# iwbn/flow-supervisor

Measured on AMD Instinct MI355X. Metric: image-pairs/s fwd+bwd, 12 GRU iters, 436x1024, higher is better.
Workload: dtype f32 (bf16x3 products); 1 GPU; RAFT full, 440x1024 (Sintel 436x1024 padded), 12 GRU iters, 4 pairs/GPU, train step = fwd + sequence loss + bwd + RCCL all-reduce + clip + AdamW; global_batch=4, parallelism=dp1, launch=hipGraph replay of the whole step

## Files before the change

flow_supervisor_amd/csrc/conv_igemm.hip:

```cpp
#include "conv_common.hpp"

namespace {

__device__ __forceinline__ void tile_of_block(int swz, int& bx, int& by) {
  if (!swz) return;
  const int nx = gridDim.x, T = nx * gridDim.y, i = by * nx + bx;
  const int x = i & 7, q = T >> 3, r = T & 7;
  const int t = x * q + (x < r ? x : r) + (i >> 3);
  bx = t % nx; by = t / nx;
}

template <class Cfg>
struct ConvALoader {
  static constexpr int BM = Cfg::BM, BK = Cfg::BK, LD = Cfg::LDA;
  static constexpr int F4 = BK / 4;
  static constexpr int NF4 = BM * F4 / 256;
  static constexpr int NREG = NF4 * 4;
  static constexpr int NCH = NF4;
  const float* p0; const float* p1; const float* p2;
  int C0, C1, C2, ld0, ld1, ld2;
  int cpt0, cpt1, cpt2;
  int taps, KW, PH, PW, H, W;
  int py[NF4], px[NF4];
  int64_t pb[NF4];
  __device__ __forceinline__ bool fetch_chunk(int kt, float (&r)[NREG], int j) const {
    const int n0 = taps * cpt0, n1 = taps * cpt1;
    const bool is1 = kt >= n0, is2 = kt >= n0 + n1;
    const int k = kt - (is1 ? n0 : 0) - (is2 ? n1 : 0);
    const int C = C0 + (is1 ? C1 - C0 : 0) + (is2 ? C2 - C1 : 0);
    const int ld = ld0 + (is1 ? ld1 - ld0 : 0) + (is2 ? ld2 - ld1 : 0);
    const int cpt = cpt0 + (is1 ? cpt1 - cpt0 : 0) + (is2 ? cpt2 - cpt1 : 0);
    const float* p = p0 + (is1 ? p1 - p0 : 0) + (is2 ? p2 - p1 : 0);
    const int tap = k / cpt, c0 = (k % cpt) * BK;
    const int dy = tap / KW - PH, dx = tap % KW - PW;
    const int kq = (threadIdx.x + 256 * j) % F4;
    const int yy = py[j] + dy, xx = px[j] + dx, c = c0 + kq * 4;
    const bool ok = py[j] >= 0 && yy >= 0 && yy < H && xx >= 0 && xx < W && c < C;
    const f32x4 v = gload4(p + (ok ? (pb[j] + (int64_t)yy * W + xx) * ld + c : 0));
    r[4 * j + 0] = v[0]; r[4 * j + 1] = v[1]; r[4 * j + 2] = v[2]; r[4 * j + 3] = v[3];
    return ok;
  }
  __device__ __forceinline__ void store_chunk(float* t, const float (&r)[NREG], int j, bool ok) const {
    const int e = threadIdx.x + 256 * j;
    const int row = e / F4, kq = e % F4;
#pragma unroll
    for (int c = 0; c < 4; ++c) t[(kq * 4 + c) * LD + row] = ok ? r[4 * j + c] : 0.f;
  }
};

template <class Cfg>
struct SplitConvALoader {
  static constexpr int NCH = Cfg::NCH_A, NREG = NCH * 4;
  const float* p0; const float* p1; const float* p2;
  int C0, C1, C2, ld0, ld1, ld2, cpt0, cpt1, cpt2;
  int taps, KW, PH, PW, H, W;
  int py[NCH], px[NCH];
  int pofs[NCH];
  __device__ __forceinline__ void fetch_chunk(int kt, float (&r)[NREG], int j) const {
    const int n0 = taps * cpt0, n1 = taps * cpt1;
    const bool is1 = kt >= n0, is2 = kt >= n0 + n1;
    const int k = kt - (is1 ? n0 : 0) - (is2 ? n1 : 0);
    const int C = C0 + (is1 ? C1 - C0 : 0) + (is2 ? C2 - C1 : 0);
    const int ld = ld0 + (is1 ? ld1 - ld0 : 0) + (is2 ? ld2 - ld1 : 0);
    const int cpt = cpt0 + (is1 ? cpt1 - cpt0 : 0) + (is2 ? cpt2 - cpt1 : 0);
    const float* p = p0 + (is1 ? p1 - p0 : 0) + (is2 ? p2 - p1 : 0);
    const int tap = k / cpt, c0 = (k % cpt) * 32;
    const int dy = tap / KW - PH, dx = tap % KW - PW;
    const int kq = (threadIdx.x + 256 * j) & 7;
    const int c = c0 + kq * 4;
    const bool ok = ((unsigned)(py[j] + dy) < (unsigned)H) && ((unsigned)(px[j] + dx) < (unsigned)W) && c < C;
    const float* src = ok ? p + (int64_t)(pofs[j] + dy * W + dx) * ld + c : g_fsraft_zero16;
    const f32x4 v = gload4(src);
    r[4 * j + 0] = v[0]; r[4 * j + 1] = v[1]; r[4 * j + 2] = v[2]; r[4 * j + 3] = v[3];
  }
  __device__ __forceinline__ void stage_chunk(char* tile, const float* r4, int j) const {
    stage_convert<Cfg::PITCH>(tile, threadIdx.x + 256 * j, r4);
  }
};

template <class Cfg>
struct BufConvALoader {
  static constexpr int NCH = Cfg::NCH_A, NREG = NCH * 4;
  const float* b0; const float* b1; const float* b2; unsigned nb0, nb1, nb2;
  unsigned ld0x4, ld1x4, ld2x4;
  const unsigned __attribute__((address_space(4)))* ktab;
  unsigned tapmask[NCH];
  unsigned pofs[NCH];
  unsigned kq16;
  __device__ __forceinline__ void fetch_tile(int kt, float (&r)[NREG]) const {
    const unsigned e = ktab[__builtin_amdgcn_readfirstlane(kt)];
    const unsigned soff = (e & 0xffffu) << 4, tap = (e >> 16) & 15u, src = (e >> 20) & 3u, crem = (e >> 22) & 63u;
    const bool s1 = src >= 1, s2 = src >= 2;
    const unsigned ldb = ld0x4 + (s1 ? ld1x4 - ld0x4 : 0u) + (s2 ? ld2x4 - ld1x4 : 0u);
    const float* bp = b0 + (s1 ? b1 - b0 : 0) + (s2 ? b2 - b1 : 0);
    const __amdgpu_buffer_rsrc_t rs = make_rsrc(bp, 0x7fffffffu);
    const unsigned cok = kq16 < crem * 4u ? 1u : 0u;
#pragma unroll
    for (int j = 0; j < NCH; ++j) {
      const unsigned bad = (__builtin_amdgcn_ubfe(tapmask[j], tap, 1u) & cok) ^ 1u;
      const unsigned voff = (bad << 31) | (__umul24(pofs[j], ldb) + kq16);
      const u32x4 v = __builtin_amdgcn_raw_buffer_load_b128(rs, voff, soff, 0);
      const f32x4 f = __builtin_bit_cast(f32x4, v);
      r[4 * j + 0] = f[0]; r[4 * j + 1] = f[1]; r[4 * j + 2] = f[2]; r[4 * j + 3] = f[3];
    }
  }
  __device__ __forceinline__ void stage_chunk(char* tile, const float* r4, int j) const {
    stage_convert<Cfg::PITCH>(tile, threadIdx.x + Cfg::NT * j, r4);
  }
};

template <class Cfg>
struct BufConvALoaderU {
  static constexpr int NCH = Cfg::NCH_A, NREG = NCH * 4;
  const float* base;
  const unsigned __attribute__((address_space(4)))* ktab;
  unsigned tapmask[NCH];
  unsigned voff0[NCH];
  unsigned kq16;
  __device__ __forceinline__ void fetch_tile(int kt, float (&r)[NREG]) const {
    const int ku = __builtin_amdgcn_readfirstlane(kt);
    const unsigned soff = ktab[2 * ku], e = ktab[2 * ku + 1];
    const unsigned tap = e & 15u, crem4 = (e >> 4) * 4u;
    const __amdgpu_buffer_rsrc_t rs = make_rsrc(base, 0x7fffffffu);
    const unsigned cok = kq16 < crem4 ? 1u : 0u;
#pragma unroll
    for (int j = 0; j < NCH; ++j) {
      const unsigned bad = (__builtin_amdgcn_ubfe(tapmask[j], tap, 1u) & cok) ^ 1u;
      const u32x4 v = __builtin_amdgcn_raw_buffer_load_b128(rs, (bad << 31) | voff0[j], soff, 0);
      const f32x4 f = __builtin_bit_cast(f32x4, v);
      r[4 * j + 0] = f[0]; r[4 * j + 1] = f[1]; r[4 * j + 2] = f[2]; r[4 * j + 3] = f[3];
    }
  }
  __device__ __forceinline__ void stage_chunk(char* tile, const float* r4, int j) const {
    stage_convert<Cfg::PITCH>(tile, threadIdx.x + Cfg::NT * j, r4);
  }
};

template <class Cfg>
struct BufWeightLoader {
  static constexpr int NCH = Cfg::NCH_B, NREG = NCH * 4;
  const char* base; unsigned nbytes;
  unsigned voff[NCH];
  __device__ __forceinline__ void fetch_tile(int kt, float (&r)[NREG]) const {
    const int ku = __builtin_amdgcn_readfirstlane(kt);
    const __amdgpu_buffer_rsrc_t rs = make_rsrc(base, ku < 0 ? 0u : nbytes);
    const unsigned soff = ku < 0 ? 0u : (unsigned)ku * 128u;
#pragma unroll
    for (int j = 0; j < NCH; ++j) {
      const u32x4 v = __builtin_amdgcn_raw_buffer_load_b128(rs, voff[j], soff, 0);
      const f32x4 f = __builtin_bit_cast(f32x4, v);
      r[4 * j + 0] = f[0]; r[4 * j + 1] = f[1]; r[4 * j + 2] = f[2]; r[4 * j + 3] = f[3];
    }
  }
  __device__ __forceinline__ void stage_chunk(char* tile, const float* r4, int j) const {
    stage_copy<Cfg::PITCH>(tile, threadIdx.x + Cfg::NT * j, r4);
  }
};

template <class Cfg>
struct SplitWeightLoader {
  static constexpr int NCH = Cfg::NCH_B, NREG = NCH * 4;
  const char* base;
  int64_t row_bytes;
  int rows_valid;
  __device__ __forceinline__ void fetch_chunk(int kt, float (&r)[NREG], int j) const {
    const int e = threadIdx.x + 256 * j;
    const int row = e >> 3, part = e & 7;
    const char* src = (row < rows_valid && kt >= 0) ? base + row * row_bytes + (int64_t)kt * 128 + part * 16
                                                    : reinterpret_cast<const char*>(g_fsraft_zero16);
    const f32x4 v = gload4(src);
    r[4 * j + 0] = v[0]; r[4 * j + 1] = v[1]; r[4 * j + 2] = v[2]; r[4 * j + 3] = v[3];
  }
  __device__ __forceinline__ void stage_chunk(char* tile, const float* r4, int j) const {
    stage_copy<Cfg::PITCH>(tile, threadIdx.x + 256 * j, r4);
  }
};

template <class Cfg, int EPI>
__device__ __forceinline__ void conv_epilogue(const ConvArgs& a, f32x16 (&acc)[Cfg::TM][Cfg::TN], int m0, int n0) {
  const int HW = a.H * a.W;
  const int M = a.B * HW;
  const int lane = threadIdx.x & 63, wave = threadIdx.x >> 6;
#pragma unroll
  for (int nt = 0; nt < Cfg::TN; ++nt) {
    const int n = n0 + acc_col<Cfg>(nt);
    const bool nok = n < a.N;
    const float bias = (nok && a.bias) ? a.bias[n] : 0.f;
    int di = 0;
    if (a.ndst > 1 && n >= a.dst[1].n0) di = 1;
    if (a.ndst > 2 && n >= a.dst[2].n0) di = 2;
    float* dp = di == 0 ? a.dst[0].p : di == 1 ? a.dst[1].p : a.dst[2].p;
    const int64_t dbs = di == 0 ? a.dst[0].bs : di == 1 ? a.dst[1].bs : a.dst[2].bs;
    const int64_t dps = di == 0 ? a.dst[0].ps : di == 1 ? a.dst[1].ps : a.dst[2].ps;
    const int64_t dcs = di == 0 ? a.dst[0].cs : di == 1 ? a.dst[1].cs : a.dst[2].cs;
    const int dn0 = di == 0 ? a.dst[0].n0 : di == 1 ? a.dst[1].n0 : a.dst[2].n0;
    const bool dacc = (di == 0 ? a.dst[0].accumulate : di == 1 ? a.dst[1].accumulate : a.dst[2].accumulate) != 0;
    const float* mk = di == 0 ? a.rmask[0] : di == 1 ? a.rmask[1] : a.rmask[2];
    const int ldm = di == 0 ? a.ldmask[0] : di == 1 ? a.ldmask[1] : a.ldmask[2];
    const int mkc = di == 0 ? a.maskc[0] : di == 1 ? a.maskc[1] : a.maskc[2];
#pragma unroll
    for (int mt = 0; mt < Cfg::TM; ++mt) {
      const int mbase = m0 + (wave / Cfg::WN) * (Cfg::TM * 32) + mt * 32 + 4 * (lane >> 5);
      const int b0 = mbase / HW, pix0 = mbase - b0 * HW;
      if (EPI == EPI_PLAIN) {
#pragma unroll
        for (int hb = 0; hb < 2; ++hb) {
          int off[8];
#pragma unroll
          for (int q = 0; q < 8; ++q) {
            const int r = hb * 8 + q;
            const int d = (r & 3) + 8 * (r >> 2);
            int pix = pix0 + d, b = b0;
            if (pix >= HW) { pix -= HW; ++b; }
            const bool ok = nok && (mbase + d < M);
            off[q] = ok ? (int)(b * dbs + pix * dps + (n - dn0) * dcs) : -1;
          }
          float old[8];
#pragma unroll
          for (int q = 0; q < 8; ++q) old[q] = (dacc && off[q] >= 0) ? dp[off[q]] : 0.f;
#pragma unroll
          for (int q = 0; q < 8; ++q) {
            float v = (acc[mt][nt][hb * 8 + q] + bias) * a.alpha;
            if (a.relu) v = fmaxf(v, 0.f);
            v += old[q];
            if (off[q] >= 0 && mk && n - dn0 < mkc) {
              const int r = hb * 8 + q;
              const int64_t m = mbase + (r & 3) + 8 * (r >> 2);
              if (mk[m * ldm + (n - dn0)] <= 0.f) v = 0.f;
            }
            if (off[q] >= 0) dp[off[q]] = v;
          }
        }
      } else if (EPI == EPI_ZR) {
        const bool isz = n < a.hid;
        const int c = isz ? n : n - a.hid;
        float hh[16];
        bool ok[16];
#pragma unroll
        for (int r = 0; r < 16; ++r) {
          const int m = mbase + (r & 3) + 8 * (r >> 2);
          ok[r] = nok && m < M;
          hh[r] = (ok[r] && !isz) ? a.h[(int64_t)m * a.ldh + c] : 0.f;
        }
#pragma unroll
        for (int r = 0; r < 16; ++r) {
          const int64_t m = mbase + (r & 3) + 8 * (r >> 2);
          const float pre = (a.pre && ok[r]) ? a.pre[m * a.ldpre + n] : 0.f;
          const float sg = 1.0f / (1.0f + expf(-(acc[mt][nt][r] + bias + pre)));
          if (ok[r]) {
            if (isz) {
              a.dst[0].p[m * a.dst[0].ps + c] = sg;
            } else {
              a.aux2[m * a.ld2 + c] = sg;
              a.aux1[m * a.ld1 + c] = sg * hh[r];
            }
          }
        }
      } else {
        float hh[16], zz[16];
        bool ok[16];
#pragma unroll
        for (int r = 0; r < 16; ++r) {
          const int64_t m = mbase + (r & 3) + 8 * (r >> 2);
          ok[r] = nok && m < M;
          hh[r] = ok[r] ? a.h[m * a.ldh + n] : 0.f;
          zz[r] = ok[r] ? a.z[m * a.ldz + n] : 0.f;
        }
#pragma unroll
        for (int r = 0; r < 16; ++r) {
          const int64_t m = mbase + (r & 3) + 8 * (r >> 2);
          const float pre = (a.pre && ok[r]) ? a.pre[m * a.ldpre + n] : 0.f;
          const float q = tanhf(acc[mt][nt][r] + bias + pre);
          if (ok[r]) {
            a.aux1[m * a.ld1 + n] = q;
            a.dst[0].p[m * a.dst[0].ps + n] = (1.f - zz[r]) * hh[r] + zz[r] * q;
          }
        }
      }
    }
  }
}

template <class Cfg, int EPI, int NTW = Cfg::NT, bool PATCH = false>
__device__ __forceinline__ void conv_epilogue_lds(const ConvArgs& a, f32x16 (&acc)[Cfg::TM][Cfg::TN], int m0, int n0,
                                                  float* __restrict__ tile, bool owner = true, int pb = 0, int py0 = 0, int px0 = 0,
                                                  int64_t mofs = 0) {
  constexpr int LD = Cfg::BN + 4;
  const int HW = a.H * a.W;
  const int M = a.B * HW;
  const int lane = threadIdx.x & 63, wave = threadIdx.x >> 6;
  auto row_m = [&](int row) -> int64_t {
    if constexpr (PATCH) {
      const int y = py0 + (row >> 5), x = px0 + (row & 31);
      return (y < a.H && x < a.W) ? (int64_t)(pb * a.H + y) * a.W + x : -1;
    } else {
      return m0 + row < M ? (int64_t)m0 + row : -1;
    }
  };
  __syncthreads();
#pragma unroll
  for (int nt = 0; nt < Cfg::TN; ++nt) {
    const int nl = acc_col<Cfg>(nt);
    const float bias = (n0 + nl < a.N && a.bias) ? a.bias[n0 + nl] : 0.f;
#pragma unroll
    for (int mt = 0; mt < Cfg::TM; ++mt) {
      const int rbase = (wave / Cfg::WN) * (Cfg::TM * 32) + mt * 32 + 4 * (lane >> 5);
#pragma unroll
      for (int r = 0; r < 16; ++r) tile[(rbase + (r & 3) + 8 * (r >> 2)) * LD + nl] = acc[mt][nt][r] + bias;
    }
  }
  __syncthreads();
  constexpr int C4 = Cfg::BN / 4;
  constexpr int RPP = NTW / C4;
  (void)owner;
  const int c4 = threadIdx.x % C4, rsub = threadIdx.x / C4;
  const int n = n0 + c4 * 4;
  const bool stats = PATCH && EPI == EPI_PLAIN && a.st_sum != nullptr;
  if (n >= a.N && !stats) return;
  if (EPI == EPI_PLAIN) {
    f32x4 ssum = {0.f, 0.f, 0.f, 0.f}, ssq = {0.f, 0.f, 0.f, 0.f};
    if (n < a.N) {
    int di = 0;
    if (a.ndst > 1 && n >= a.dst[1].n0) di = 1;
    if (a.ndst > 2 && n >= a.dst[2].n0) di = 2;
    float* dp = di == 0 ? a.dst[0].p : di == 1 ? a.dst[1].p : a.dst[2].p;
    const int64_t dps = di == 0 ? a.dst[0].ps : di == 1 ? a.dst[1].ps : a.dst[2].ps;
    const int dn0 = di == 0 ? a.dst[0].n0 : di == 1 ? a.dst[1].n0 : a.dst[2].n0;
    const bool dacc = (di == 0 ? a.dst[0].accumulate : di == 1 ? a.dst[1].accumulate : a.dst[2].accumulate) != 0;
    const float* mk = di == 0 ? a.rmask[0] : di == 1 ? a.rmask[1] : a.rmask[2];
    const int ldm = di == 0 ? a.ldmask[0] : di == 1 ? a.ldmask[1] : a.ldmask[2];
    const int mkc = di == 0 ? a.maskc[0] : di == 1 ? a.maskc[1] : a.maskc[2];
    const int nv = a.N - n < 4 ? a.N - n : 4;
#pragma unroll 4
    for (int row = rsub; row < Cfg::BM; row += RPP) {
      const int64_t m = row_m(row);
      if (m < 0) { if (PATCH) continue; else break; }
      f32x4 v = *reinterpret_cast<const f32x4*>(tile + row * LD + c4 * 4);
      float* o = dp + (int64_t)(m + mofs) * dps + (n - dn0);
#pragma unroll
      for (int i = 0; i < 4; ++i) {
        v[i] *= a.alpha;
        if (a.relu) v[i] = fmaxf(v[i], 0.f);
      }
      if (nv == 4) {
        if (stats) { ssum += v; ssq += v * v; }
        if (dacc) {
          const f32x4 old = gload4(o);
#pragma unroll
          for (int i = 0; i < 4; ++i) v[i] += old[i];
        }
        if (mk) {
          const f32x4 y = gload4(mk + (int64_t)m * ldm + (n - dn0));
#pragma unroll
          for (int i = 0; i < 4; ++i) if (n - dn0 + i < mkc && y[i] <= 0.f) v[i] = 0.f;
        }
        gstore4(o, v);
      } else {
        for (int i = 0; i < nv; ++i) {
          float r = dacc ? gload1(o + i) + v[i] : v[i];
          if (mk && n - dn0 + i < mkc && gload1(mk + (int64_t)m * ldm + (n - dn0) + i) <= 0.f) r = 0.f;
          gstore1(o + i, r);
        }
      }
    }
    }
    if constexpr (PATCH) {
      if (stats) {
        __syncthreads();
        float* red = tile;
        *reinterpret_cast<f32x4*>(red + (rsub * Cfg::BN) + c4 * 4) = ssum;
        *reinterpret_cast<f32x4*>(red + ((RPP + rsub) * Cfg::BN) + c4 * 4) = ssq;
        __syncthreads();
        if (threadIdx.x < Cfg::BN && n0 + (int)threadIdx.x < a.N) {
          float t1 = 0.f, t2 = 0.f;
#pragma unroll 4
          for (int g = 0; g < RPP; ++g) { t1 += red[g * Cfg::BN + threadIdx.x]; t2 += red[(RPP + g) * Cfg::BN + threadIdx.x]; }
          const int64_t o = ((int64_t)pb * a.st_slots + (int)(blockIdx.y % (unsigned)a.st_slots)) * a.N + n0 + threadIdx.x;
          atomicAdd(a.st_sum + o, t1);
          atomicAdd(a.st_sq + o, t2);
        }
      }
    }
  } else if (EPI == EPI_ZR) {
    const bool isz = n < a.hid;
    const int c = isz ? n : n - a.hid;
#pragma unroll 4
    for (int row = rsub; row < Cfg::BM; row += RPP) {
      const int64_t mr = row_m(row);
      if (mr < 0 && !PATCH) break;
      const int64_t m = mr < 0 ? 0 : mr;
      f32x4 v = *reinterpret_cast<const f32x4*>(tile + row * LD + c4 * 4);
      if (a.pre) v += gload4(a.pre + m * a.ldpre + n);
      f32x4 hh = {0.f, 0.f, 0.f, 0.f};
      if (!isz) hh = gload4(a.h + m * a.ldh + c);
#pragma unroll
      for (int i = 0; i < 4; ++i) v[i] = 1.0f / (1.0f + expf(-v[i]));
      if (mr < 0) continue;
      if (isz) {
        *reinterpret_cast<f32x4*>(a.dst[0].p + m * a.dst[0].ps + c) = v;
      } else {
        *reinterpret_cast<f32x4*>(a.aux2 + m * a.ld2 + c) = v;
        f32x4 rh;
#pragma unroll
        for (int i = 0; i < 4; ++i) rh[i] = v[i] * hh[i];
        *reinterpret_cast<f32x4*>(a.aux1 + m * a.ld1 + c) = rh;
      }
    }
  } else {
#pragma unroll 4
    for (int row = rsub; row < Cfg::BM; row += RPP) {
      const int64_t m = row_m(row);
      if (m < 0) { if (PATCH) continue; else break; }
      f32x4 v = *reinterpret_cast<const f32x4*>(tile + row * LD + c4 * 4);
      if (a.pre) v += gload4(a.pre + m * a.ldpre + n);
      const f32x4 hh = gload4(a.h + m * a.ldh + n);
      const f32x4 zz = gload4(a.z + m * a.ldz + n);
      f32x4 hn;
#pragma unroll
      for (int i = 0; i < 4; ++i) {
        v[i] = tanhf(v[i]);
        hn[i] = (1.f - zz[i]) * hh[i] + zz[i] * v[i];
      }
      *reinterpret_cast<f32x4*>(a.aux1 + m * a.ld1 + n) = v;
      *reinterpret_cast<f32x4*>(a.dst[0].p + m * a.dst[0].ps + n) = hn;
    }
  }
}

__device__ __forceinline__ bool epilogue_rows_ok(const ConvArgs& a) {
  bool ok = true;
  for (int i = 0; i < a.ndst; ++i)
    ok = ok && a.dst[i].cs == 1 && (a.dst[i].ps & 3) == 0 && (a.dst[i].n0 & 3) == 0 && ((uintptr_t)a.dst[i].p & 15) == 0 &&
         a.dst[i].bs == a.dst[i].ps * (int64_t)(a.H * a.W);
  return ok;
}

bool epilogue_rows_ok_host(const ConvArgs& a) {
  bool ok = true;
  for (int i = 0; i < a.ndst; ++i)
    ok = ok && a.dst[i].cs == 1 && (a.dst[i].ps & 3) == 0 && (a.dst[i].n0 & 3) == 0 && ((uintptr_t)a.dst[i].p & 15) == 0 &&
         a.dst[i].bs == a.dst[i].ps * (int64_t)(a.H * a.W);
  return ok;
}

template <class Cfg, int EPI>
__global__ __launch_bounds__(256) void conv_igemm_kernel(ConvArgs a) {
  __shared__ __attribute__((aligned(16))) float lds[Cfg::LDS_FLOATS];
  const int HW = a.H * a.W;
  const int M = a.B * HW;
  const int n0 = blockIdx.x * Cfg::BN, m0 = blockIdx.y * Cfg::BM;
  ConvALoader<Cfg> la;
  la.p0 = a.src[0].p; la.C0 = a.src[0].C; la.ld0 = a.src[0].ld; la.cpt0 = (a.src[0].C + 31) / 32 * (32 / Cfg::BK);
  la.p1 = a.src[1].p; la.C1 = a.src[1].C; la.ld1 = a.src[1].ld; la.cpt1 = a.nsrc > 1 ? (a.src[1].C + 31) / 32 * (32 / Cfg::BK) : 0;
  la.p2 = a.src[2].p; la.C2 = a.src[2].C; la.ld2 = a.src[2].ld; la.cpt2 = a.nsrc > 2 ? (a.src[2].C + 31) / 32 * (32 / Cfg::BK) : 0;
  if (a.nsrc < 2) { la.p1 = a.src[0].p; la.C1 = 0; la.ld1 = 4; la.cpt1 = 1; }
  if (a.nsrc < 3) { la.p2 = a.src[0].p; la.C2 = 0; la.ld2 = 4; la.cpt2 = 1; }
  la.taps = a.KH * a.KW; la.KW = a.KW; la.PH = a.PH; la.PW = a.PW; la.H = a.H; la.W = a.W;
#pragma unroll
  for (int j = 0; j < ConvALoader<Cfg>::NF4; ++j) {
    const int row = (threadIdx.x + 256 * j) / ConvALoader<Cfg>::F4;
    const int m = m0 + row;
    if (m < M) {
      const int b = m / HW, pix = m % HW;
      la.py[j] = pix / a.W; la.px[j] = pix % a.W; la.pb[j] = (int64_t)b * HW;
    } else {
      la.py[j] = -1; la.px[j] = 0; la.pb[j] = 0;
    }
  }
  RowMajorTileLoader<Cfg::BN, Cfg::BK, Cfg::LDB> lb{a.wpk + (int64_t)n0 * a.Ktot, a.Ktot, a.N - n0, a.Ktot};
  f32x16 acc[Cfg::TM][Cfg::TN];
#pragma unroll
  for (int i = 0; i < Cfg::TM; ++i)
#pragma unroll
    for (int j = 0; j < Cfg::TN; ++j)
#pragma unroll
      for (int r = 0; r < 16; ++r) acc[i][j][r] = 0.f;
  gemm_mainloop<Cfg>(lds, a.Ktot / Cfg::BK, la, lb, acc);
  conv_epilogue<Cfg, EPI>(a, acc, m0, n0);
}

template <class Cfg, int EPI, int BUF = 0>
__global__ __launch_bounds__(Cfg::NT) void conv_igemm_split_kernel(const std::conditional_t<BUF != 0, ConvArgsT, ConvArgs> args) {
  static_assert(Cfg::NT == 256 || BUF != 0, "wider workgroups use the buffer-addressed loaders");
  __shared__ __attribute__((aligned(16))) char lds[Cfg::LDS_ALLOC];
  const ConvArgs& a = [&]() -> const ConvArgs& { if constexpr (BUF != 0) return args.a; else return args; }();
  const int HW = a.H * a.W;
  const int M = a.B * HW;
  int bx = blockIdx.x, by = blockIdx.y;
  tile_of_block(a.swz, bx, by);
  const int n0 = bx * Cfg::BN, m0 = by * Cfg::BM;
  f32x16 acc[Cfg::TM][Cfg::TN];
#pragma unroll
  for (int i = 0; i < Cfg::TM; ++i)
#pragma unroll
    for (int j = 0; j < Cfg::TN; ++j)
#pragma unroll
      for (int r = 0; r < 16; ++r) acc[i][j][r] = 0.f;
  if constexpr (BUF != 0) {
    const int PH = a.PH, PW = a.PW, taps = a.KH * a.KW;
    const auto* ktab = (const unsigned __attribute__((address_space(4)))*)(
        (const char __attribute__((address_space(4)))*)__builtin_amdgcn_kernarg_segment_ptr() + offsetof(ConvArgsT, ktab));
    int kt0 = 0, KTs = a.Ktot / 32;
    if (a.ksplit > 1) {
      const int per = (KTs + a.ksplit - 1) / a.ksplit;
      kt0 = (int)blockIdx.z * per;
      KTs = min(per, KTs - kt0);
      ktab += kt0 * (BUF >= 2 ? 2 : 1);
    }
    unsigned tapmask[Cfg::NCH_A], pofs[Cfg::NCH_A];
#pragma unroll
    for (int j = 0; j < Cfg::NCH_A; ++j) {
      const int m = m0 + ((threadIdx.x + Cfg::NT * j) >> 3);
      unsigned mask = 0;
      if (m < M) {
        const int pix = m % HW, y = pix / a.W, x = pix % a.W;
        for (int t = 0; t < taps; ++t) {
          const int yy = y + t / a.KW - PH, xx = x + t % a.KW - PW;
          if ((unsigned)yy < (unsigned)a.H && (unsigned)xx < (unsigned)a.W) mask |= 1u << t;
        }
      }
      tapmask[j] = mask; pofs[j] = m < M ? m : 0;
    }
    BufWeightLoader<Cfg> lb;
    lb.base = uni_ptr(reinterpret_cast<const char*>(a.wpk) + (int64_t)n0 * a.Ktot * 4 + (int64_t)kt0 * 128);
    lb.nbytes = 0x7fffffffu;
#pragma unroll
    for (int j = 0; j < BufWeightLoader<Cfg>::NCH; ++j) {
      const int e = threadIdx.x + Cfg::NT * j;
      lb.voff[j] = (e >> 3) < a.N - n0 ? (unsigned)((e >> 3) * a.Ktot * 4 + (e & 7) * 16) : FS_OOB;
    }
    if constexpr (BUF >= 2) {
      BufConvALoaderU<Cfg> la;
      la.base = uni_ptr(args.ubase); la.ktab = ktab; la.kq16 = (threadIdx.x & 7) * 16;
      const unsigned ldb = uni((unsigned)args.uld * 4u);
#pragma unroll
      for (int j = 0; j < Cfg::NCH_A; ++j) { la.tapmask[j] = tapmask[j]; la.voff0[j] = pofs[j] * ldb + la.kq16; }
      split_mainloop<Cfg, BufConvALoaderU<Cfg>, BufWeightLoader<Cfg>, true>(lds, KTs, la, lb, acc);
    } else {
      BufConvALoader<Cfg> la;
      la.ld0x4 = uni(a.src[0].ld * 4); la.ld1x4 = uni(a.src[1].ld * 4); la.ld2x4 = uni(a.src[2].ld * 4);
      la.b0 = uni_ptr(a.src[0].p - (int64_t)(PH * a.W + PW) * a.src[0].ld); la.nb0 = 0x7fffffffu;
      la.b1 = uni_ptr(a.src[1].p - (int64_t)(PH * a.W + PW) * a.src[1].ld); la.nb1 = 0x7fffffffu;
      la.b2 = uni_ptr(a.src[2].p - (int64_t)(PH * a.W + PW) * a.src[2].ld); la.nb2 = 0x7fffffffu;
      la.ktab = ktab;
      la.kq16 = (threadIdx.x & 7) * 16;
#pragma unroll
      for (int j = 0; j < Cfg::NCH_A; ++j) { la.tapmask[j] = tapmask[j]; la.pofs[j] = pofs[j]; }
      split_mainloop<Cfg, BufConvALoader<Cfg>, BufWeightLoader<Cfg>, true>(lds, KTs, la, lb, acc);
    }
    if constexpr (EPI == EPI_PLAIN && Cfg::LDS_ALLOC >= Cfg::BM * (Cfg::BN + 4) * 4) {
      if (a.ksplit > 1) {
        conv_epilogue_lds<Cfg, EPI_PLAIN>(a, acc, m0, n0, reinterpret_cast<float*>(lds), true, 0, 0, 0, (int64_t)blockIdx.z * M);
        return;
      }
    }
  } else {
  SplitConvALoader<Cfg> la;
  la.p0 = a.src[0].p; la.C0 = a.src[0].C; la.ld0 = a.src[0].ld; la.cpt0 = (a.src[0].C + 31) / 32;
  la.p1 = a.src[1].p; la.C1 = a.src[1].C; la.ld1 = a.src[1].ld; la.cpt1 = a.nsrc > 1 ? (a.src[1].C + 31) / 32 : 0;
  la.p2 = a.src[2].p; la.C2 = a.src[2].C; la.ld2 = a.src[2].ld; la.cpt2 = a.nsrc > 2 ? (a.src[2].C + 31) / 32 : 0;
  if (a.nsrc < 2) { la.p1 = a.src[0].p; la.C1 = 0; la.ld1 = 4; la.cpt1 = 1; }
  if (a.nsrc < 3) { la.p2 = a.src[0].p; la.C2 = 0; la.ld2 = 4; la.cpt2 = 1; }
  la.taps = a.KH * a.KW; la.KW = a.KW; la.PH = a.PH; la.PW = a.PW; la.H = a.H; la.W = a.W;
#pragma unroll
  for (int j = 0; j < SplitConvALoader<Cfg>::NCH; ++j) {
    const int m = m0 + ((threadIdx.x + 256 * j) >> 3);
    if (m < M) {
      const int pix = m % HW;
      la.py[j] = pix / a.W; la.px[j] = pix % a.W; la.pofs[j] = m;
    } else {
      la.py[j] = -(1 << 20); la.px[j] = 0; la.pofs[j] = 0;
    }
  }
  SplitWeightLoader<Cfg> lb{reinterpret_cast<const char*>(a.wpk) + (int64_t)n0 * a.Ktot * 4, (int64_t)a.Ktot * 4, a.N - n0};
  split_mainloop<Cfg>(lds, a.Ktot / 32, la, lb, acc);
  }
  if constexpr (Cfg::LDS_ALLOC >= Cfg::BM * (Cfg::BN + 4) * 4) {
    if (EPI != EPI_PLAIN || epilogue_rows_ok(a)) {
      conv_epilogue_lds<Cfg, EPI>(a, acc, m0, n0, reinterpret_cast<float*>(lds));
      return;
    }
  }
  conv_epilogue<Cfg, EPI>(a, acc, m0, n0);
}

constexpr int HALO_TH = 4, HALO_TW = 32, HALO_PW = HALO_TW + 2, HALO_ROWS = (HALO_TH + 2) * HALO_PW;
struct HaloArgs {
  const float* x; int ldx, C;
  const char* wpk;
  const float* bias;
  float* out; int64_t obs, ops;
  int N, B, H, W, relu;
  int acc;
  float* st_sum; float* st_sq; int st_slots;
};

template <int CG, int TN>
__global__ __launch_bounds__(256) void conv3x3_halo_kernel(const HaloArgs a) {
  constexpr int PLANE = HALO_ROWS * 128;
  constexpr int NCHH = (HALO_ROWS * CG * 8 + 255) / 256, KT = 9 * CG;
  __shared__ __attribute__((aligned(16))) char lds[CG * PLANE];
  const int lane = threadIdx.x & 63, wave = threadIdx.x >> 6;
  const int wm = wave >> 1, wn = wave & 1, l31 = lane & 31, lh = lane >> 5;
  const int x0 = blockIdx.x * HALO_TW, y0 = blockIdx.y * HALO_TH, b = blockIdx.z;

  const int NB = (a.N + 31) >> 5;
  const char* wbase = uni_ptr(a.wpk);
  struct BFrag { u32x4 v[TN][4]; };
  auto fetch_b = [&](int kt, BFrag& f) {
    const int ku = __builtin_amdgcn_readfirstlane(kt < KT ? kt : KT - 1);
    const __amdgpu_buffer_rsrc_t rs = make_rsrc(wbase, 0x7fffffffu);
#pragma unroll
    for (int nt = 0; nt < TN; ++nt) {
      const int nb = wn * TN + nt;
      const unsigned soff = (unsigned)((ku * NB + (nb < NB ? nb : 0)) * 4096);
      const unsigned voff = nb < NB ? (unsigned)lane * 16u : FS_OOB;
#pragma unroll
      for (int q = 0; q < 4; ++q) f.v[nt][q] = __builtin_amdgcn_raw_buffer_load_b128(rs, voff, soff + 1024u * q, 0);
    }
  };
  BFrag f[4];
  fetch_b(0, f[0]);
  fetch_b(1, f[1]);
  fetch_b(2, f[2]);

  {
    const float* img = uni_ptr(a.x + (int64_t)b * a.H * a.W * a.ldx);
    const __amdgpu_buffer_rsrc_t rs = make_rsrc(img, 0x7fffffffu);
    float rh[NCHH * 4];
#pragma unroll
    for (int j = 0; j < NCHH; ++j) {
      const int e = threadIdx.x + 256 * j;
      const int row = e / (CG * 8), rem = e % (CG * 8), ch = (rem >> 3) * 32 + (rem & 7) * 4;
      const int y = y0 - 1 + row / HALO_PW, x = x0 - 1 + row % HALO_PW;
      const bool ok = row < HALO_ROWS && (unsigned)y < (unsigned)a.H && (unsigned)x < (unsigned)a.W && ch < a.C;
      const unsigned voff = ok ? (unsigned)((y * a.W + x) * a.ldx + ch) * 4u : FS_OOB;
      const f32x4 f = __builtin_bit_cast(f32x4, __builtin_amdgcn_raw_buffer_load_b128(rs, voff, 0, 0));
      rh[4 * j + 0] = f[0]; rh[4 * j + 1] = f[1]; rh[4 * j + 2] = f[2]; rh[4 * j + 3] = f[3];
    }
#pragma unroll
    for (int j = 0; j < NCHH; ++j) {
      const int e = threadIdx.x + 256 * j;
      const int row = e / (CG * 8), rem = e % (CG * 8);
      if (row < HALO_ROWS) stage_convert<128>(lds + (rem >> 3) * PLANE, row * 8 + (rem & 7), rh + 4 * j);
    }
  }
  __syncthreads();

  f32x16 acc[2][TN];
#pragma unroll
  for (int i = 0; i < 2; ++i)
#pragma unroll
    for (int j = 0; j < TN; ++j)
#pragma unroll
      for (int r = 0; r < 16; ++r) acc[i][j][r] = 0.f;

  auto compute = [&](int kt, const BFrag& f) {
    const int ku = __builtin_amdgcn_readfirstlane(kt);
    const int tap = ku / CG, g = ku - tap * CG, dy = tap / 3, dx = tap - dy * 3;
    const char* Ap = lds + g * PLANE;
    const int rowa = (2 * wm + dy) * HALO_PW + dx + l31;
#pragma unroll
    for (int s = 0; s < 2; ++s) {
      bf16x8 ah[2], al[2];
#pragma unroll
      for (int mt = 0; mt < 2; ++mt) {
        const int row = rowa + mt * HALO_PW;
        ah[mt] = *reinterpret_cast<const bf16x8*>(Ap + slot_offset<128>(row, 2 * s + lh));
        al[mt] = *reinterpret_cast<const bf16x8*>(Ap + slot_offset<128>(row, 4 + 2 * s + lh));
      }
#pragma unroll
      for (int mt = 0; mt < 2; ++mt)
#pragma unroll
        for (int nt = 0; nt < TN; ++nt) {
          const bf16x8 bh = __builtin_bit_cast(bf16x8, f.v[nt][s]), bl = __builtin_bit_cast(bf16x8, f.v[nt][2 + s]);
          acc[mt][nt] = __builtin_amdgcn_mfma_f32_32x32x16_bf16(al[mt], bh, acc[mt][nt], 0, 0, 0);
// ... 434 lines not shown
```

flow_supervisor_amd/csrc/conv_patch.inc:

```
constexpr int PT_TW = 32, PT_BN = 128;
constexpr int PT_GMAX = 32;

struct PatchArgs {
  ConvArgs a;
  int ngroups;
  int tx;
  unsigned gtab[PT_GMAX];
  int cpt[3];
};

template <int EPI, int KH, int KW, int PT_TH, int BN = PT_BN>
__global__ __launch_bounds__(PT_TH * 64) void conv_patch_kernel(const PatchArgs args) {
  constexpr int PT_NT = PT_TH * 64, TN = BN / 64;
  using PCfg = SplitCfg<PT_TH * 32, BN, PT_TH / 2, 2, 2, true, PT_NT>;
  constexpr int TAPS = KH * KW, PHh = KH / 2, PWh = KW / 2;
  constexpr int PH = PT_TH + KH - 1, PW = PT_TW + KW - 1, ROWS = PH * PW;
  constexpr int PPITCH = 144;
  constexpr int PT_PLANE = ROWS * PPITCH;
  constexpr int PT_NCHP = (ROWS * 8 + PT_NT - 1) / PT_NT;
  constexpr int EPI_BYTES = PT_TH * 32 * (BN + 4) * 4, RING = 2 * PT_PLANE + 2 * BN * 128;
  __shared__ __attribute__((aligned(16))) char lds[RING > EPI_BYTES ? RING : EPI_BYTES];
  const ConvArgs& a = args.a;
  const int lane = threadIdx.x & 63, wave = __builtin_amdgcn_readfirstlane((int)(threadIdx.x >> 6));
  const int wm = wave >> 1, wn = wave & 1, l31 = lane & 31, lh = lane >> 5;
  const int n0 = blockIdx.x * BN;
  const int tile = blockIdx.y, tpi = args.tx * ((a.H + PT_TH - 1) / PT_TH);
  const int b = tile / tpi, trem = tile % tpi;
  const int y0 = (trem / args.tx) * PT_TH, x0 = (trem % args.tx) * PT_TW;
  const auto* gtab = (const unsigned __attribute__((address_space(4)))*)(
      (const char __attribute__((address_space(4)))*)__builtin_amdgcn_kernarg_segment_ptr() + offsetof(PatchArgs, gtab));
  const int NG = args.ngroups;

  unsigned ppix[PT_NCHP];
  const unsigned part16 = (threadIdx.x & 7) * 16;
#pragma unroll
  for (int j = 0; j < PT_NCHP; ++j) {
    const int row = (threadIdx.x + PT_NT * j) >> 3;
    const int y = y0 - PHh + row / PW, x = x0 - PWh + row % PW;
    const bool ok = row < ROWS && (unsigned)y < (unsigned)a.H && (unsigned)x < (unsigned)a.W;
    ppix[j] = ok ? (unsigned)((b * a.H + y) * a.W + x) : 0x7fffffffu;
  }
  constexpr int NCHW = BN * 8 / PT_NT;
  unsigned vbw[NCHW];
#pragma unroll
  for (int j = 0; j < NCHW; ++j) {
    const int e = threadIdx.x + PT_NT * j;
    vbw[j] = (e >> 3) < a.N - n0 ? (unsigned)((e >> 3) * a.Ktot * 4 + (e & 7) * 16) : FS_OOB;
  }
  const char* wbase = uni_ptr(reinterpret_cast<const char*>(a.wpk) + (int64_t)n0 * a.Ktot * 4);

  struct Group { const float* base; unsigned ld4, soff, crem4; int kt0, step; };
  auto group = [&](int g) {
    const unsigned e = gtab[__builtin_amdgcn_readfirstlane(g < NG ? g : NG - 1)];
    const unsigned src = e & 3u, c = (e >> 2) & 255u, crem = (e >> 10) & 63u;
    const bool s1 = src >= 1, s2 = src >= 2;
    Group r;
    r.base = uni_ptr(a.src[0].p + (s1 ? a.src[1].p - a.src[0].p : 0) + (s2 ? a.src[2].p - a.src[1].p : 0));
    r.ld4 = uni((unsigned)(a.src[0].ld + (s1 ? a.src[1].ld - a.src[0].ld : 0) + (s2 ? a.src[2].ld - a.src[1].ld : 0)) * 4u);
    r.soff = c * 128u; r.crem4 = crem * 4u;
    r.kt0 = (int)(e >> 16);
    r.step = args.cpt[0] + (s1 ? args.cpt[1] - args.cpt[0] : 0) + (s2 ? args.cpt[2] - args.cpt[1] : 0);
    return r;
  };
  float rp[PT_NCHP * 4];
  auto fetch_patch = [&](const Group& gr) {
    const __amdgpu_buffer_rsrc_t rs = make_rsrc(gr.base, 0x7fffffffu);
    const unsigned cok = part16 < gr.crem4 ? 0u : 0x80000000u;
#pragma unroll
    for (int j = 0; j < PT_NCHP; ++j) {
      const unsigned voff = ppix[j] == 0x7fffffffu ? FS_OOB : ((ppix[j] * gr.ld4 + part16) | cok);
      const f32x4 f = __builtin_bit_cast(f32x4, __builtin_amdgcn_raw_buffer_load_b128(rs, voff, gr.soff, 0));
      rp[4 * j] = f[0]; rp[4 * j + 1] = f[1]; rp[4 * j + 2] = f[2]; rp[4 * j + 3] = f[3];
    }
  };
  auto stage_patch = [&](char* plane) {
#pragma unroll
    for (int j = 0; j < PT_NCHP; ++j) {
      const int e = threadIdx.x + PT_NT * j;
      if ((e >> 3) < ROWS) stage_convert<PPITCH>(plane, e, rp + 4 * j);
    }
  };
  const __amdgpu_buffer_rsrc_t rsW = make_rsrc(wbase, 0x7fffffffu);
  float rw[NCHW * 4];
  auto fetch_w = [&](int kt) {
    const int ku = __builtin_amdgcn_readfirstlane(kt);
#pragma unroll
    for (int j = 0; j < NCHW; ++j) {
      const f32x4 f = __builtin_bit_cast(f32x4, __builtin_amdgcn_raw_buffer_load_b128(rsW, ku < 0 ? FS_OOB : vbw[j], ku < 0 ? 0u : (unsigned)ku * 128u, 0));
      rw[4 * j] = f[0]; rw[4 * j + 1] = f[1]; rw[4 * j + 2] = f[2]; rw[4 * j + 3] = f[3];
    }
  };
  auto stage_w = [&](char* bt) {
#pragma unroll
    for (int j = 0; j < NCHW; ++j) stage_copy<128>(bt, threadIdx.x + PT_NT * j, rw + 4 * j);
  };

  f32x16 acc[2][TN];
#pragma unroll
  for (int i = 0; i < 2; ++i)
#pragma unroll
    for (int j = 0; j < TN; ++j)
#pragma unroll
      for (int r = 0; r < 16; ++r) acc[i][j][r] = 0.f;
  char* plane0 = lds;
  char* plane1 = lds + PT_PLANE;
  char* bt0 = lds + 2 * PT_PLANE;
  char* bt1 = bt0 + BN * 128;

  const int rb = wn * (BN / 2) + l31;
  const int la_off = (2 * wm * PW + l31) * PPITCH + lh * 16;
  auto compute = [&](const char* plane, const char* bt, int dy, int dx) {
    const char* Bs = bt + rb * 128;
#pragma unroll
    for (int s = 0; s < 2; ++s) {
      bf16x8 ah[2], al[2], bh[TN], bl[TN];
#pragma unroll
      for (int mt = 0; mt < 2; ++mt) {
        ah[mt] = *reinterpret_cast<const bf16x8*>(plane + la_off + ((dy + mt) * PW + dx) * PPITCH + (2 * s) * 16);
        al[mt] = *reinterpret_cast<const bf16x8*>(plane + la_off + ((dy + mt) * PW + dx) * PPITCH + (4 + 2 * s) * 16);
      }
      const int obh = slot_offset<128>(rb, 2 * s + lh) - rb * 128, obl = slot_offset<128>(rb, 4 + 2 * s + lh) - rb * 128;
#pragma unroll
      for (int nt = 0; nt < TN; ++nt) {
        bh[nt] = *reinterpret_cast<const bf16x8*>(Bs + nt * 32 * 128 + obh);
        bl[nt] = *reinterpret_cast<const bf16x8*>(Bs + nt * 32 * 128 + obl);
      }
#pragma unroll
      for (int mt = 0; mt < 2; ++mt)
#pragma unroll
        for (int nt = 0; nt < TN; ++nt) acc[mt][nt] = __builtin_amdgcn_mfma_f32_32x32x16_bf16(al[mt], bh[nt], acc[mt][nt], 0, 0, 0);
#pragma unroll
      for (int mt = 0; mt < 2; ++mt)
#pragma unroll
        for (int nt = 0; nt < TN; ++nt) acc[mt][nt] = __builtin_amdgcn_mfma_f32_32x32x16_bf16(ah[mt], bl[nt], acc[mt][nt], 0, 0, 0);
#pragma unroll
      for (int mt = 0; mt < 2; ++mt)
#pragma unroll
        for (int nt = 0; nt < TN; ++nt) acc[mt][nt] = __builtin_amdgcn_mfma_f32_32x32x16_bf16(ah[mt], bh[nt], acc[mt][nt], 0, 0, 0);
    }
  };

  Group gc = group(0);
  fetch_patch(gc);
  fetch_w(gc.kt0);
  stage_patch(plane0);
  stage_w(bt0);
  Group gn = group(1);
  if (NG > 1) fetch_patch(gn);
  fetch_w(TAPS > 1 ? gc.kt0 + gc.step : (NG > 1 ? gn.kt0 : -1));
  __syncthreads();
  for (int g = 0; g < NG; ++g) {
#pragma unroll
    for (int t = 0; t < TAPS; ++t) {
      const int i = g * TAPS + t;
      char* btc = (i & 1) ? bt1 : bt0;
      char* btn = (i & 1) ? bt0 : bt1;
      compute((g & 1) ? plane1 : plane0, btc, t / KW, t % KW);
      stage_w(btn);
      {
        const int t2 = t + 2;
        int kt;
        if (t2 < TAPS) kt = gc.kt0 + t2 * gc.step;
        else kt = g + 1 < NG ? gn.kt0 + (t2 - TAPS) * gn.step : -1;
        if (TAPS == 1) {
          const Group g2 = group(g + 2);
          kt = g + 2 < NG ? g2.kt0 : -1;
        }
        fetch_w(kt);
      }
      if (t == TAPS - 1 && g + 1 < NG) {
        stage_patch((g & 1) ? plane0 : plane1);
        gc = gn;
        gn = group(g + 2);
        if (g + 2 < NG) fetch_patch(gn);
      }
      __syncthreads();
    }
  }
  conv_epilogue_lds<PCfg, EPI, PT_NT, true>(a, acc, 0, n0, reinterpret_cast<float*>(lds), true, b, y0, x0);
}

template <int KH, int KW, int TH>
int launch_conv_patch_t(const PatchArgs& p, int epi, dim3 grid, hipStream_t s) {
  t_route[0] = (TH == 8 ? 11 : 10) + (KH == 3 && KW == 3 && p.a.N <= 64 ? 2 : 0);
  if constexpr (KH == 3 && KW == 3) {
    if (p.a.N <= 64) {
      hipLaunchKernelGGL((conv_patch_kernel<EPI_PLAIN, 3, 3, TH, 64>), grid, dim3(TH * 64), 0, s, p);
      return fs_launch_status();
    }
  }
  with_epi(epi, [&](auto e) { hipLaunchKernelGGL((conv_patch_kernel<decltype(e)::value, KH, KW, TH>), grid, dim3(TH * 64), 0, s, p); });
  return fs_launch_status();
}

int launch_conv_patch(const ConvArgs& a, int epi, hipStream_t s) {
  const bool k33 = a.KH == 3 && a.KW == 3, k15 = a.KH == 1 && a.KW == 5, k51 = a.KH == 5 && a.KW == 1;
  if (!(k33 || k15 || k51) || a.PH != a.KH / 2 || a.PW != a.KW / 2 || !epilogue_rows_ok_host(a)) return -1;
  PatchArgs p;
  p.a = a; p.a.swz = 0;
  int ng = 0, kt = 0;
  const int taps = a.KH * a.KW;
  for (int sidx = 0; sidx < 3; ++sidx) p.cpt[sidx] = 1;
  for (int sidx = 0; sidx < a.nsrc; ++sidx) {
    const int C = a.src[sidx].C, cpt = (C + 31) / 32;
    p.cpt[sidx] = cpt;
    if ((int64_t)a.B * a.H * a.W * a.src[sidx].ld * 4 >= (int64_t)0x7fffffff) return -1;
    for (int c = 0; c < cpt; ++c) {
      if (ng >= PT_GMAX || kt + c >= (1 << 16)) return -1;
      const int crem = C - c * 32 < 32 ? C - c * 32 : 32;
      p.gtab[ng++] = (unsigned)sidx | (unsigned)c << 2 | (unsigned)crem << 10 | (unsigned)(kt + c) << 16;
    }
    kt += taps * cpt;
  }
  if (kt * 32 != a.Ktot || ng < 1) return -1;
  for (int g = ng; g < PT_GMAX; ++g) p.gtab[g] = p.gtab[ng - 1];
  p.ngroups = ng;
  p.tx = ceil_div(a.W, PT_TW);
  const int bn = a.N <= 64 ? 64 : PT_BN;
  if (bn == 64 && !(k33 && epi == EPI_PLAIN)) return -1;
  const int64_t wg8 = (int64_t)ceil_div(a.N, bn) * p.tx * ceil_div(a.H, 8) * a.B;
  if (bn == 64 && wg8 >= 200 && knob.conv_patch64 == 1) return -1;
  if (wg8 >= 200 && !(bn == 64 && knob.conv_patch64 == 2)) {
    dim3 grid(ceil_div(a.N, bn), p.tx * ceil_div(a.H, 8) * a.B);
    if (k33) return launch_conv_patch_t<3, 3, 8>(p, epi, grid, s);
    if (k15) return launch_conv_patch_t<1, 5, 8>(p, epi, grid, s);
    return launch_conv_patch_t<5, 1, 8>(p, epi, grid, s);
  }
  const bool small_grid_33 = k33 && a.N > 128 && (int64_t)ceil_div(a.N, 128) * ceil_div(a.B * a.H * a.W, 128) > 120;
  if (knob.conv_patch != 2 && bn != 64 && !small_grid_33) return -1;
  dim3 grid(ceil_div(a.N, bn), p.tx * ceil_div(a.H, 4) * a.B);
  if (k33) return launch_conv_patch_t<3, 3, 4>(p, epi, grid, s);
  if (k15) return launch_conv_patch_t<1, 5, 4>(p, epi, grid, s);
  return launch_conv_patch_t<5, 1, 4>(p, epi, grid, s);
}
```

Baseline: 110.1 image-pairs/s.

## Balance N columns across patch-conv blocks and skip MFMAs on dead column tiles

The patch conv kernel now spreads output channels evenly across column blocks (ncols rounded to 32) instead of fixed 128-wide blocks. Each wave computes how many 32-column subtiles are live and specialises the K loop to run full, one, or zero MFMA subtiles, so waves holding padded channels stop issuing matrix work. It also swizzles the wave-to-tile mapping for the 8-row variant and passes the wave index and column cap into the epilogue. This adds three template instantiations of the main loop, which raises code size and may raise register pressure. The column bound now has to be applied consistently in the epilogue.

```diff
diff --git a/flow_supervisor_amd/csrc/conv_igemm.hip b/flow_supervisor_amd/csrc/conv_igemm.hip
--- a/flow_supervisor_amd/csrc/conv_igemm.hip
+++ b/flow_supervisor_amd/csrc/conv_igemm.hip
@@ -284,11 +284,12 @@
 template <class Cfg, int EPI, int NTW = Cfg::NT, bool PATCH = false>
 __device__ __forceinline__ void conv_epilogue_lds(const ConvArgs& a, f32x16 (&acc)[Cfg::TM][Cfg::TN], int m0, int n0,
                                                   float* __restrict__ tile, bool owner = true, int pb = 0, int py0 = 0, int px0 = 0,
-                                                  int64_t mofs = 0) {
+                                                  int64_t mofs = 0, int pwave = -1, int ncap = 0x7fffffff) {
   constexpr int LD = Cfg::BN + 4;
   const int HW = a.H * a.W;
   const int M = a.B * HW;
-  const int lane = threadIdx.x & 63, wave = threadIdx.x >> 6;
+  const int lane = threadIdx.x & 63, wave = (PATCH && pwave >= 0) ? pwave : (int)(threadIdx.x >> 6);
+  const int nend = a.N < ncap ? a.N : ncap;
   auto row_m = [&](int row) -> int64_t {
     if constexpr (PATCH) {
       const int y = py0 + (row >> 5), x = px0 + (row & 31);
@@ -300,8 +301,9 @@
   __syncthreads();
 #pragma unroll
   for (int nt = 0; nt < Cfg::TN; ++nt) {
-    const int nl = acc_col<Cfg>(nt);
-    const float bias = (n0 + nl < a.N && a.bias) ? a.bias[n0 + nl] : 0.f;
+    const int nb0 = (wave % Cfg::WN) * (Cfg::TN * 32) + nt * 32, nl = nb0 + (lane & 31);
+    if (PATCH && n0 + nb0 >= nend) continue;
+    const float bias = (n0 + nl < nend && a.bias) ? a.bias[n0 + nl] : 0.f;
 #pragma unroll
     for (int mt = 0; mt < Cfg::TM; ++mt) {
       const int rbase = (wave / Cfg::WN) * (Cfg::TM * 32) + mt * 32 + 4 * (lane >> 5);
@@ -316,10 +318,10 @@
   const int c4 = threadIdx.x % C4, rsub = threadIdx.x / C4;
   const int n = n0 + c4 * 4;
   const bool stats = PATCH && EPI == EPI_PLAIN && a.st_sum != nullptr;
-  if (n >= a.N && !stats) return;
+  if (n >= nend && !stats) return;
   if (EPI == EPI_PLAIN) {
     f32x4 ssum = {0.f, 0.f, 0.f, 0.f}, ssq = {0.f, 0.f, 0.f, 0.f};
-    if (n < a.N) {
+    if (n < nend) {
     int di = 0;
     if (a.ndst > 1 && n >= a.dst[1].n0) di = 1;
     if (a.ndst > 2 && n >= a.dst[2].n0) di = 2;
@@ -330,7 +332,7 @@
     const float* mk = di == 0 ? a.rmask[0] : di == 1 ? a.rmask[1] : a.rmask[2];
     const int ldm = di == 0 ? a.ldmask[0] : di == 1 ? a.ldmask[1] : a.ldmask[2];
     const int mkc = di == 0 ? a.maskc[0] : di == 1 ? a.maskc[1] : a.maskc[2];
-    const int nv = a.N - n < 4 ? a.N - n : 4;
+    const int nv = nend - n < 4 ? nend - n : 4;
 #pragma unroll 4
     for (int row = rsub; row < Cfg::BM; row += RPP) {
       const int64_t m = row_m(row);
@@ -371,7 +373,7 @@
         *reinterpret_cast<f32x4*>(red + (rsub * Cfg::BN) + c4 * 4) = ssum;
         *reinterpret_cast<f32x4*>(red + ((RPP + rsub) * Cfg::BN) + c4 * 4) = ssq;
         __syncthreads();
-        if (threadIdx.x < Cfg::BN && n0 + (int)threadIdx.x < a.N) {
+        if (threadIdx.x < Cfg::BN && n0 + (int)threadIdx.x < nend) {
           float t1 = 0.f, t2 = 0.f;
 #pragma unroll 4
           for (int g = 0; g < RPP; ++g) { t1 += red[g * Cfg::BN + threadIdx.x]; t2 += red[(RPP + g) * Cfg::BN + threadIdx.x]; }
diff --git a/flow_supervisor_amd/csrc/conv_patch.inc b/flow_supervisor_amd/csrc/conv_patch.inc
--- a/flow_supervisor_amd/csrc/conv_patch.inc
+++ b/flow_supervisor_amd/csrc/conv_patch.inc
@@ -5,6 +5,7 @@
   ConvArgs a;
   int ngroups;
   int tx;
+  int ncols;
   unsigned gtab[PT_GMAX];
   int cpt[3];
 };
@@ -22,8 +23,12 @@
   __shared__ __attribute__((aligned(16))) char lds[RING > EPI_BYTES ? RING : EPI_BYTES];
   const ConvArgs& a = args.a;
   const int lane = threadIdx.x & 63, wave = __builtin_amdgcn_readfirstlane((int)(threadIdx.x >> 6));
-  const int wm = wave >> 1, wn = wave & 1, l31 = lane & 31, lh = lane >> 5;
-  const int n0 = blockIdx.x * BN;
+  const int lw = (PT_TH == 8 && BN == 128) ? wave ^ ((wave >> 2) & 1) : wave;
+  const int wm = lw >> 1, wn = lw & 1, l31 = lane & 31, lh = lane >> 5;
+  const int ncols = BN == 128 ? args.ncols : BN;
+  const int n0 = blockIdx.x * ncols;
+  const int nlive = a.N - n0 < ncols ? a.N - n0 : ncols;
+  const int ntv = BN == 128 ? __builtin_amdgcn_readfirstlane(min(max((nlive - wn * 64 + 31) >> 5, 0), TN)) : TN;
   const int tile = blockIdx.y, tpi = args.tx * ((a.H + PT_TH - 1) / PT_TH);
   const int b = tile / tpi, trem = tile % tpi;
   const int y0 = (trem / args.tx) * PT_TH, x0 = (trem % args.tx) * PT_TW;
@@ -45,7 +50,7 @@
 #pragma unroll
   for (int j = 0; j < NCHW; ++j) {
     const int e = threadIdx.x + PT_NT * j;
-    vbw[j] = (e >> 3) < a.N - n0 ? (unsigned)((e >> 3) * a.Ktot * 4 + (e & 7) * 16) : FS_OOB;
+    vbw[j] = (e >> 3) < nlive ? (unsigned)((e >> 3) * a.Ktot * 4 + (e & 7) * 16) : FS_OOB;
   }
   const char* wbase = uni_ptr(reinterpret_cast<const char*>(a.wpk) + (int64_t)n0 * a.Ktot * 4);
 
@@ -109,11 +114,12 @@
 
   const int rb = wn * (BN / 2) + l31;
   const int la_off = (2 * wm * PW + l31) * PPITCH + lh * 16;
-  auto compute = [&](const char* plane, const char* bt, int dy, int dx) {
+  auto compute_n = [&](auto nv_c, const char* plane, const char* bt, int dy, int dx) {
+    constexpr int NV = decltype(nv_c)::value;
     const char* Bs = bt + rb * 128;
 #pragma unroll
     for (int s = 0; s < 2; ++s) {
-      bf16x8 ah[2], al[2], bh[TN], bl[TN];
+      bf16x8 ah[2], al[2], bh[NV], bl[NV];
 #pragma unroll
       for (int mt = 0; mt < 2; ++mt) {
         ah[mt] = *reinterpret_cast<const bf16x8*>(plane + la_off + ((dy + mt) * PW + dx) * PPITCH + (2 * s) * 16);
@@ -121,22 +127,22 @@
       }
       const int obh = slot_offset<128>(rb, 2 * s + lh) - rb * 128, obl = slot_offset<128>(rb, 4 + 2 * s + lh) - rb * 128;
 #pragma unroll
-      for (int nt = 0; nt < TN; ++nt) {
+      for (int nt = 0; nt < NV; ++nt) {
         bh[nt] = *reinterpret_cast<const bf16x8*>(Bs + nt * 32 * 128 + obh);
         bl[nt] = *reinterpret_cast<const bf16x8*>(Bs + nt * 32 * 128 + obl);
       }
 #pragma unroll
       for (int mt = 0; mt < 2; ++mt)
 #pragma unroll
-        for (int nt = 0; nt < TN; ++nt) acc[mt][nt] = __builtin_amdgcn_mfma_f32_32x32x16_bf16(al[mt], bh[nt], acc[mt][nt], 0, 0, 0);
+        for (int nt = 0; nt < NV; ++nt) acc[mt][nt] = __builtin_amdgcn_mfma_f32_32x32x16_bf16(al[mt], bh[nt], acc[mt][nt], 0, 0, 0);
 #pragma unroll
       for (int mt = 0; mt < 2; ++mt)
 #pragma unroll
-        for (int nt = 0; nt < TN; ++nt) acc[mt][nt] = __builtin_amdgcn_mfma_f32_32x32x16_bf16(ah[mt], bl[nt], acc[mt][nt], 0, 0, 0);
+        for (int nt = 0; nt < NV; ++nt) acc[mt][nt] = __builtin_amdgcn_mfma_f32_32x32x16_bf16(ah[mt], bl[nt], acc[mt][nt], 0, 0, 0);
 #pragma unroll
       for (int mt = 0; mt < 2; ++mt)
 #pragma unroll
-        for (int nt = 0; nt < TN; ++nt) acc[mt][nt] = __builtin_amdgcn_mfma_f32_32x32x16_bf16(ah[mt], bh[nt], acc[mt][nt], 0, 0, 0);
+        for (int nt = 0; nt < NV; ++nt) acc[mt][nt] = __builtin_amdgcn_mfma_f32_32x32x16_bf16(ah[mt], bh[nt], acc[mt][nt], 0, 0, 0);
     }
   };
 
@@ -149,35 +155,40 @@
   if (NG > 1) fetch_patch(gn);
   fetch_w(TAPS > 1 ? gc.kt0 + gc.step : (NG > 1 ? gn.kt0 : -1));
   __syncthreads();
-  for (int g = 0; g < NG; ++g) {
-#pragma unroll
-    for (int t = 0; t < TAPS; ++t) {
-      const int i = g * TAPS + t;
-      char* btc = (i & 1) ? bt1 : bt0;
-      char* btn = (i & 1) ? bt0 : bt1;
-      compute((g & 1) ? plane1 : plane0, btc, t / KW, t % KW);
-      stage_w(btn);
-      {
-        const int t2 = t + 2;
-        int kt;
-        if (t2 < TAPS) kt = gc.kt0 + t2 * gc.step;
-        else kt = g + 1 < NG ? gn.kt0 + (t2 - TAPS) * gn.step : -1;
-        if (TAPS == 1) {
-          const Group g2 = group(g + 2);
-          kt = g + 2 < NG ? g2.kt0 : -1;
+  auto kloop = [&](auto nv_c) {
+    for (int g = 0; g < NG; ++g) {
+#pragma unroll
+      for (int t = 0; t < TAPS; ++t) {
+        const int i = g * TAPS + t;
+        char* btc = (i & 1) ? bt1 : bt0;
+        char* btn = (i & 1) ? bt0 : bt1;
+        if constexpr (decltype(nv_c)::value > 0) compute_n(nv_c, (g & 1) ? plane1 : plane0, btc, t / KW, t % KW);
+        stage_w(btn);
+        {
+          const int t2 = t + 2;
+          int kt;
+          if (t2 < TAPS) kt = gc.kt0 + t2 * gc.step;
+          else kt = g + 1 < NG ? gn.kt0 + (t2 - TAPS) * gn.step : -1;
+          if (TAPS == 1) {
+            const Group g2 = group(g + 2);
+            kt = g + 2 < NG ? g2.kt0 : -1;
+          }
+          fetch_w(kt);
         }
-        fetch_w(kt);
+        if (t == TAPS - 1 && g + 1 < NG) {
+          stage_patch((g & 1) ? plane0 : plane1);
+          gc = gn;
+          gn = group(g + 2);
+          if (g + 2 < NG) fetch_patch(gn);
+        }
+        __syncthreads();
       }
-      if (t == TAPS - 1 && g + 1 < NG) {
-        stage_patch((g & 1) ? plane0 : plane1);
-        gc = gn;
-        gn = group(g + 2);
-        if (g + 2 < NG) fetch_patch(gn);
-      }
-      __syncthreads();
-    }
-  }
-  conv_epilogue_lds<PCfg, EPI, PT_NT, true>(a, acc, 0, n0, reinterpret_cast<float*>(lds), true, b, y0, x0);
+    }
+  };
+  if (ntv == TN) kloop(std::integral_constant<int, TN>{});
+  else if (TN > 1 && ntv == 1) kloop(std::integral_constant<int, 1>{});
+  else kloop(std::integral_constant<int, 0>{});
+  conv_epilogue_lds<PCfg, EPI, PT_NT, true>(a, acc, 0, n0, reinterpret_cast<float*>(lds), true, b, y0, x0, 0, lw, n0 + ncols);
 }
 
 template <int KH, int KW, int TH>
@@ -217,6 +228,8 @@
   p.ngroups = ng;
   p.tx = ceil_div(a.W, PT_TW);
   const int bn = a.N <= 64 ? 64 : PT_BN;
+  const int nbt = ceil_div(a.N, bn);
+  p.ncols = bn == 64 ? 64 : 32 * ceil_div(ceil_div(a.N, 32), nbt);
   if (bn == 64 && !(k33 && epi == EPI_PLAIN)) return -1;
   const int64_t wg8 = (int64_t)ceil_div(a.N, bn) * p.tx * ceil_div(a.H, 8) * a.B;
   if (bn == 64 && wg8 >= 200 && knob.conv_patch64 == 1) return -1;
```

Result: no change. 110.7 image-pairs/s, median of 6 (+0.6%).
